# srbittner/torch_nf

Measured on AMD Instinct MI355X. Metric: M samples/sec NormFlow.log_prob, D=64 RealNVPx8, N=2^20, higher is better.
Workload: dtype f32

## Files before the change

torch_nf_amd/csrc/f16_tile2.h:

```cpp
#pragma once
#ifndef TNF2_ABL
#define TNF2_ABL 0
#endif
#if TNF2_ABL == 4
#define TNF_SPLIT_RNE_NO_REMAINDER 1
#endif
#include "f16_tile.h"
#include "support_math.h"

#ifndef TNF2_SCHED
#define TNF2_SCHED 0
#endif

namespace tnf {


typedef __bf16 bf2 __attribute__((ext_vector_type(2)));
typedef __bf16 bf8 __attribute__((ext_vector_type(8)));
typedef short s4 __attribute__((ext_vector_type(4)));
__device__ __forceinline__ unsigned pk_bf16(float a, float b) {
    return __builtin_bit_cast(unsigned, __builtin_convertvector(f2{a, b}, bf2));
}
__device__ __forceinline__ f4 mfma16b(u2 a, u2 b, f4 c) {
    return __builtin_amdgcn_mfma_f32_16x16x16bf16_1k(__builtin_bit_cast(s4, a), __builtin_bit_cast(s4, b), c, 0, 0, 0);
}
__device__ __forceinline__ f4 mfma32b(u4 a, u4 b, f4 c) {
    return __builtin_amdgcn_mfma_f32_16x16x32_bf16(__builtin_bit_cast(bf8, a), __builtin_bit_cast(bf8, b), c, 0, 0, 0);
}

__device__ __forceinline__ f4 contract16(u4 wv, h4 rh, h4 rl, f4 c) {
    const h4 wh = __builtin_bit_cast(h4, u2{wv[0], wv[1]}), wl = __builtin_bit_cast(h4, u2{wv[2], wv[3]});
    return mfma16h(wl, rh, mfma16h(wh, rl, mfma16h(wh, rh, c)));
}

__device__ __forceinline__ float sig2s(float a, float S) {
#if TNF2_ABL == 1
    return __builtin_fmaf(a, S, S);
#else
    return __builtin_amdgcn_rcpf(__builtin_fmaf(__builtin_amdgcn_exp2f(a), S, S));
#endif
}
__device__ __forceinline__ f4 sig2s_4(f4 v, float S) {
    return f4{sig2s(v[0], S), sig2s(v[1], S), sig2s(v[2], S), sig2s(v[3], S)};
}

template <int H, int L>
struct Img2 {
    static constexpr int HT = H / 16;
    static constexpr int N0 = (H == 32) ? 4 : 0;
    static constexpr int NK = ((H == 16) ? 2 : 0) + 2 * (L - 1) + 2 * HT;
    static constexpr int NBG = 2 + 2 * (L - 1) + 2 * HT;
    static constexpr int OFF_D = N0 * 256;
    static constexpr int OFF_B = OFF_D + NK * 256;
    static constexpr int OFF_S = OFF_B + NBG * 16;
    static constexpr int OFF_A = OFF_S + 8;
    static constexpr int FLOATS = OFF_A + 2 * H;
    __device__ static constexpr int k_l0(int net) { return net; }
    __device__ static constexpr int k_h(int l, int net) { return ((H == 16) ? 2 : 0) + 2 * l + net; }
    __device__ static constexpr int k_o(int net, int mo) { return ((H == 16) ? 2 : 0) + 2 * (L - 1) + net * HT + mo; }
    __device__ static constexpr int b_b0(int net) { return net; }
    __device__ static constexpr int b_bh(int l, int net) { return 2 + 2 * l + net; }
    __device__ static constexpr int b_b2(int net, int mo) { return 2 + 2 * (L - 1) + net * HT + mo; }
};
static_assert(Img2<32, 3>::FLOATS % 4 == 0 && Img2<16, 1>::FLOATS % 4 == 0, "images must stay 16-byte aligned");

template <int H>
__device__ __forceinline__ int layer_kappa(const float* __restrict__ p, int U, int lane, const float* foldc, int c,
                                           int din = H) {
    constexpr int D = 2 * H;
    constexpr int HT = H / 16;
    const int r = lane & 15, q = lane >> 4;
    const int coff = (c & 1) ? H : 0;
    const float* wt = p;
    const float* ws = p + din * U;
    float mx = 0.f;
#pragma unroll
    for (int m = 0; m < HT; ++m)
#pragma unroll
        for (int j = 0; j < 4; ++j) {
            const int f = 16 * m + 4 * q + j;
            const bool ok = r < U && f < din;
            const float a = foldc[coff + f];
            mx = fmaxf(mx, fabsf(kTwoLog2e * ld_sel(wt, f * U + r, ok) * a));
            mx = fmaxf(mx, fabsf(kTwoLog2e * ld_sel(ws, f * U + r, ok) * a));
        }
    (void)D;
    return pow2_norm(wave_max(mx), -30, 30);
}

template <int PREC>
__device__ __forceinline__ void store_k16(u4* gd, const float (&v)[4]) {
    if constexpr (PREC == 1) {
        *gd = u4{pk_bf16(v[0], v[1]), pk_bf16(v[2], v[3]), 0u, 0u};
    } else {
        const HiLo a = split2r(v[0], v[1]), b = split2r(v[2], v[3]);
        *gd = u4{a.hi, b.hi, a.lo, b.lo};
    }
}

template <int H, int L, int PREC = 0, bool FWD = false>
__device__ __forceinline__ void build_image2(float* img, const float* __restrict__ p, int U, int lane, const float* foldc,
                                             const float* foldprev, int c, float sc_in, float sc_prev, float sig_next,
                                             int din = H, int dout = H) {
    typedef Img2<H, L> I;
    constexpr int D = 2 * H;
    constexpr int HT = I::HT;
    LayerW<H, L> w;
    load_layer_w<H, L>(w, p, U, lane, din, dout);
    const int q = lane >> 4;
    const int coff = (c & 1) ? H : 0, toff = (c & 1) ? 0 : H;

#pragma unroll
    for (int net = 0; net < 2; ++net) {
        float pb = 0.f;
#pragma unroll
        for (int m = 0; m < HT; ++m)
#pragma unroll
            for (int j = 0; j < 4; ++j) {
                const int f = 16 * m + 4 * q + j;
                pb = __builtin_fmaf(w.w0[net][m * 4 + j], foldc[D + coff + f], pb);
                w.w0[net][m * 4 + j] *= foldc[coff + f] * sc_in;
            }
        pb = reduce_q(pb);
#pragma unroll
        for (int j = 0; j < 4; ++j) w.b0[net][j] += __shfl(pb, 4 * q + j);
    }
    float Sst[L][2];
#pragma unroll
    for (int l = 0; l < L - 1; ++l)
// ... 21 lines not shown
            if constexpr (FWD) w.b2[0][mo][j] *= sig_next;
            else w.b2[0][mo][j] = (w.b2[0][mo][j] - __builtin_fmaf(Ac, Bp, Bc)) * sig_next;
        }
#pragma unroll
    for (int net = 0; net < 2; ++net) {
        float mx = 0.f;
#pragma unroll
        for (int mo = 0; mo < HT; ++mo)
#pragma unroll
            for (int j = 0; j < 4; ++j) {
                if (net == 0) w.w2[0][mo][j] *= sig_next;
                mx = fmaxf(mx, fabsf(w.w2[net][mo][j]));
            }
        const float S = pow2i(pow2_norm(wave_max(mx), -15, 40));
        Sst[L - 1][net] = S;
#pragma unroll
        for (int mo = 0; mo < HT; ++mo)
#pragma unroll
            for (int j = 0; j < 4; ++j) w.w2[net][mo][j] *= S;
    }

    u4* g0 = reinterpret_cast<u4*>(img) + lane;
    u4* gd = reinterpret_cast<u4*>(img + I::OFF_D) + lane;
#pragma unroll
    for (int net = 0; net < 2; ++net) {
        if constexpr (H == 32) {
            u4 hi, lo;
#pragma unroll
            for (int pp = 0; pp < 4; ++pp) {
                if constexpr (PREC == 1) {
                    hi[pp] = pk_bf16(w.w0[net][2 * pp], w.w0[net][2 * pp + 1]);
                    lo[pp] = 0u;
                } else {
                    const HiLo s = split2r(w.w0[net][2 * pp], w.w0[net][2 * pp + 1]);
                    hi[pp] = s.hi;
                    lo[pp] = s.lo;
                }
            }
            g0[(2 * net) * 64] = hi;
            g0[(2 * net + 1) * 64] = lo;
        } else {
            const float v[4] = {w.w0[net][0], w.w0[net][1], w.w0[net][2], w.w0[net][3]};
            store_k16<PREC>(gd + I::k_l0(net) * 64, v);
        }
#pragma unroll
        for (int l = 0; l < L - 1; ++l) {
// ... 4 lines not shown
        for (int mo = 0; mo < HT; ++mo) {
            const float v[4] = {w.w2[net][mo][0], w.w2[net][mo][1], w.w2[net][mo][2], w.w2[net][mo][3]};
            store_k16<PREC>(gd + I::k_o(net, mo) * 64, v);
        }
    }
    if ((lane & 15) == 0) {
        float* bl = img + I::OFF_B + q * 4;
#pragma unroll
        for (int net = 0; net < 2; ++net) {
            *reinterpret_cast<f4*>(bl + I::b_b0(net) * 16) = w.b0[net];
#pragma unroll
            for (int l = 0; l < L - 1; ++l) *reinterpret_cast<f4*>(bl + I::b_bh(l, net) * 16) = w.bh[l][net];
#pragma unroll
            for (int mo = 0; mo < HT; ++mo) *reinterpret_cast<f4*>(bl + I::b_b2(net, mo) * 16) = w.b2[net][mo];
        }
#pragma unroll
        for (int mo = 0; mo < HT; ++mo) {
            *reinterpret_cast<f4*>(img + I::OFF_A + 16 * mo + 4 * q) = ays[mo];
            *reinterpret_cast<f4*>(img + I::OFF_A + H + 16 * mo + 4 * q) = bys[mo];
        }
    }
    if (lane == 0) {
#pragma unroll
        for (int l = 0; l < 4; ++l) {
            img[I::OFF_S + 2 * l] = l < L ? Sst[l < L ? l : 0][0] : 1.f;
            img[I::OFF_S + 2 * l + 1] = l < L ? Sst[l < L ? l : 0][1] : 1.f;
        }
    }
}

template <int H, int L, int NT>
__device__ __forceinline__ void coupling_tile2_bf16(const float* img, int lane, const f4 (&x)[NT][H / 16], f4 (&y)[NT][H / 16],
                                                    float (&ssum2)[NT]) {
    typedef Img2<H, L> I;
    constexpr int HT = I::HT;
    const u4* g0 = reinterpret_cast<const u4*>(img) + lane;
    const u4* gd = reinterpret_cast<const u4*>(img + I::OFF_D) + lane;
    const float* bl = img + I::OFF_B + (lane >> 4) * 4;
    auto bias = [&](int g) -> f4 { return *reinterpret_cast<const f4*>(bl + g * 16); };
    auto w16 = [&](int g) -> u2 { const u4 v = gd[g * 64]; return u2{v[0], v[1]}; };
    const f4 Sa = *reinterpret_cast<const f4*>(img + I::OFF_S);
    f4 Sb = {1.f, 1.f, 1.f, 1.f};
    if constexpr (L == 3) Sb = *reinterpret_cast<const f4*>(img + I::OFF_S + 4);
    auto Sc = [&](int stage, int net) -> float { return (2 * stage + net) < 4 ? Sa[2 * stage + net] : Sb[2 * stage + net - 4]; };
    auto b4 = [&](f4 v) -> u2 { return u2{pk_bf16(v[0], v[1]), pk_bf16(v[2], v[3])}; };

    f4 acc[NT][2];
// ... 24 lines not shown
        for (int t = 0; t < NT; ++t)
#pragma unroll
            for (int net = 0; net < 2; ++net) {
                acc[t][net] = mfma16b(w16(I::k_h(l, net)), rb[t][net], bias(I::b_bh(l, net)));
                rb[t][net] = b4(sig2s_4(acc[t][net], Sc(l + 1, net)));
            }
    }
#pragma unroll
    for (int mo = 0; mo < HT; ++mo) {
        const f4 ay = *reinterpret_cast<const f4*>(img + I::OFF_A + 16 * mo + 4 * (lane >> 4));
#pragma unroll
        for (int t = 0; t < NT; ++t) {
            const f4 tt = mfma16b(w16(I::k_o(0, mo)), rb[t][0], bias(I::b_b2(0, mo)));
            const f4 sv = mfma16b(w16(I::k_o(1, mo)), rb[t][1], bias(I::b_b2(1, mo)));
#pragma unroll
            for (int j = 0; j < 4; ++j) {
                ssum2[t] += sv[j];
                y[t][mo][j] = __builtin_fmaf(y[t][mo][j], ay[j], -tt[j]) * __builtin_amdgcn_exp2f(-sv[j]);
            }
        }
    }
}

template <int H, int L, int NT, bool SLOW, int PREC = 0, bool FWD = false>
__device__ __forceinline__ void coupling_tile2(const float* img, int lane, const f4 (&x)[NT][H / 16], f4 (&y)[NT][H / 16],
                                               float (&ssum2)[NT]) {
    static_assert(!(FWD && PREC == 1), "the bf16 experiment covers the inverse direction");
    if constexpr (PREC == 1) {
        coupling_tile2_bf16<H, L, NT>(img, lane, x, y, ssum2);
        return;
    }
    typedef Img2<H, L> I;
    constexpr int HT = I::HT;
#if TNF2_SCHED == 3 || TNF2_SCHED == 4
    __builtin_amdgcn_sched_barrier(0);
#elif TNF2_SCHED == 1
    __builtin_amdgcn_iglp_opt(0);
#elif TNF2_SCHED == 2
    __builtin_amdgcn_iglp_opt(1);
#endif
    const u4* g0 = reinterpret_cast<const u4*>(img) + lane;
    const u4* gd = reinterpret_cast<const u4*>(img + I::OFF_D) + lane;
    const float* bl = img + I::OFF_B + (lane >> 4) * 4;
    auto bias = [&](int g) -> f4 { return *reinterpret_cast<const f4*>(bl + g * 16); };
    const f4 Sa = *reinterpret_cast<const f4*>(img + I::OFF_S);
    f4 Sb = {1.f, 1.f, 1.f, 1.f};
    if constexpr (L == 3) Sb = *reinterpret_cast<const f4*>(img + I::OFF_S + 4);
    auto Sc = [&](int stage, int net) -> float { return (2 * stage + net) < 4 ? Sa[2 * stage + net] : Sb[2 * stage + net - 4]; };

    f4 acc[NT][2];
    if constexpr (!SLOW) {
        if constexpr (H == 32) {
            h8 xh[NT], xl[NT];
#pragma unroll
            for (int t = 0; t < NT; ++t) {
                const HiLo a = split2r(x[t][0][0], x[t][0][1]), b = split2r(x[t][0][2], x[t][0][3]);
                const HiLo c = split2r(x[t][1][0], x[t][1][1]), d = split2r(x[t][1][2], x[t][1][3]);
                xh[t] = __builtin_bit_cast(h8, u4{a.hi, b.hi, c.hi, d.hi});
                xl[t] = __builtin_bit_cast(h8, u4{a.lo, b.lo, c.lo, d.lo});
            }
#pragma unroll
            for (int net = 0; net < 2; ++net) {
                const h8 wh = __builtin_bit_cast(h8, g0[(2 * net) * 64]);
                const h8 wl = __builtin_bit_cast(h8, g0[(2 * net + 1) * 64]);
                const f4 b0 = bias(I::b_b0(net));
#pragma unroll
                for (int t = 0; t < NT; ++t) acc[t][net] = mfma32h(wh, xh[t], b0);
#pragma unroll
                for (int t = 0; t < NT; ++t) acc[t][net] = mfma32h(wh, xl[t], acc[t][net]);
#pragma unroll
                for (int t = 0; t < NT; ++t) acc[t][net] = mfma32h(wl, xh[t], acc[t][net]);
            }
        } else {
            h4 xh[NT], xl[NT];
#pragma unroll
            for (int t = 0; t < NT; ++t) split4r(x[t][0], xh[t], xl[t]);
#pragma unroll
            for (int net = 0; net < 2; ++net) {
                const u4 wv = gd[I::k_l0(net) * 64];
                const f4 b0 = bias(I::b_b0(net));
#pragma unroll
                for (int t = 0; t < NT; ++t) acc[t][net] = contract16(wv, xh[t], xl[t], b0);
            }
        }
    } else {
#pragma unroll
        for (int net = 0; net < 2; ++net) {
            float wv[H / 4];
            if constexpr (H == 32) {
                const h8 wh = __builtin_bit_cast(h8, g0[(2 * net) * 64]);
                const h8 wl = __builtin_bit_cast(h8, g0[(2 * net + 1) * 64]);
#pragma unroll
                for (int i = 0; i < 8; ++i) wv[i] = (float)wh[i] + (float)wl[i];
            } else {
                const h8 wd = __builtin_bit_cast(h8, gd[I::k_l0(net) * 64]);
#pragma unroll
                for (int i = 0; i < 4; ++i) wv[i] = (float)wd[i] + (float)wd[4 + i];
            }
            const f4 b0 = bias(I::b_b0(net));
// ... 4 lines not shown
#pragma unroll
                for (int t = 0; t < NT; ++t) acc[t][net] = mfma4(wv[i], x[t][i >> 2][i & 3], acc[t][net]);
        }
    }
    h4 rh[NT][2], rl[NT][2];
#pragma unroll
    for (int t = 0; t < NT; ++t)
#pragma unroll
        for (int net = 0; net < 2; ++net) split4r(sig2s_4(acc[t][net], Sc(0, net)), rh[t][net], rl[t][net]);
#pragma unroll
    for (int l = 0; l < L - 1; ++l) {
#pragma unroll
        for (int net = 0; net < 2; ++net) {
            const u4 wv = gd[I::k_h(l, net) * 64];
            const f4 bh = bias(I::b_bh(l, net));
#pragma unroll
            for (int t = 0; t < NT; ++t) acc[t][net] = contract16(wv, rh[t][net], rl[t][net], bh);
        }
#pragma unroll
        for (int t = 0; t < NT; ++t)
#pragma unroll
            for (int net = 0; net < 2; ++net) split4r(sig2s_4(acc[t][net], Sc(l + 1, net)), rh[t][net], rl[t][net]);
    }
#pragma unroll
    for (int mo = 0; mo < HT; ++mo) {
        f4 tt[NT], sv[NT];
        {
            const u4 wv = gd[I::k_o(0, mo) * 64];
            const f4 b2 = bias(I::b_b2(0, mo));
#pragma unroll
            for (int t = 0; t < NT; ++t) tt[t] = contract16(wv, rh[t][0], rl[t][0], b2);
        }
        {
            const u4 wv = gd[I::k_o(1, mo) * 64];
            const f4 b2 = bias(I::b_b2(1, mo));
#pragma unroll
            for (int t = 0; t < NT; ++t) sv[t] = contract16(wv, rh[t][1], rl[t][1], b2);
        }
        const f4 ay = *reinterpret_cast<const f4*>(img + I::OFF_A + 16 * mo + 4 * (lane >> 4));
        f4 by = {0.f, 0.f, 0.f, 0.f};
        if constexpr (FWD) by = *reinterpret_cast<const f4*>(img + I::OFF_A + H + 16 * mo + 4 * (lane >> 4));
#pragma unroll
        for (int t = 0; t < NT; ++t)
#pragma unroll
            for (int j = 0; j < 4; ++j) {
                const float s2 = sv[t][j];
#if TNF2_ABL == 3
                if (j == 0 && mo == 0) ssum2[t] += s2;
#else
                ssum2[t] += s2;
#endif
                if constexpr (FWD)
                    y[t][mo][j] = __builtin_fmaf(__builtin_fmaf(y[t][mo][j], ay[j], by[j]), __builtin_amdgcn_exp2f(s2), tt[t][j]);
                else
                    y[t][mo][j] = __builtin_fmaf(y[t][mo][j], ay[j], -tt[t][j]) * __builtin_amdgcn_exp2f(-s2);
            }
    }
#if TNF2_SCHED == 3 || TNF2_SCHED == 4
    constexpr int NMFMA = NT * 3 * (2 + 2 * (L - 1) + 2 * HT);
#pragma unroll
    for (int i = 0; i < NMFMA; ++i) {
        __builtin_amdgcn_sched_group_barrier(0x008, 1, 0);
#if TNF2_SCHED == 3
        __builtin_amdgcn_sched_group_barrier(0x002, 5, 0);
#else
        __builtin_amdgcn_sched_group_barrier(0x400, 2, 0);
        __builtin_amdgcn_sched_group_barrier(0x002, 3, 0);
#endif
    }
#endif
}

}
```

torch_nf_amd/csrc/flow_fused2.hip:

```cpp
#include <type_traits>

#include "f16_tile2.h"
#include "launch.h"

#ifndef TNF2_NT
#define TNF2_NT 2
#endif
#ifndef TNF2_NW
#define TNF2_NW 8
#endif
#ifndef TNF2_NW16
#define TNF2_NW16 12
#endif
#ifndef TNF2_RANGE_NT
#define TNF2_RANGE_NT 2
#endif
#ifndef TNF2_RANGE_NW
#define TNF2_RANGE_NW 8
#endif
#ifndef TNF2_RANGE_WGPC
#define TNF2_RANGE_WGPC 1
#endif
#ifndef TNF2_RANGE_ABL
#define TNF2_RANGE_ABL 0
// ... 12 lines not shown
#endif
#ifndef TNF2_RANGE_ALT
#define TNF2_RANGE_ALT 1
#endif
#ifndef TNF2_RANGE_NTMEM
#define TNF2_RANGE_NTMEM 2
#endif
#ifndef TNF2_FUSED_STAGE
#define TNF2_FUSED_STAGE 1
#endif
#ifndef TNF2_STAMP
#define TNF2_STAMP 0
#endif
#ifndef TNF2_UNROLL
#define TNF2_UNROLL 1
#endif
#ifndef TNF2_PAD_UNROLL32
#define TNF2_PAD_UNROLL32 0
#endif

namespace tnf {


template <int H, int L>
__host__ __device__ constexpr int flow2_lds_floats(int nl) {
    return nl * Img2<H, L>::FLOATS + (nl + 1) * 4 * H + 4 * H + ((nl + 3) / 4) * 4 + 4 + 16 + 7 * 2 * H;
}

template <int H, int L, int NT, int SS, bool SLOW, bool FWD = false>
__device__ __forceinline__ void run_layers2(const float* img, int S, int lane, f4 (&lo)[NT][H / 16], f4 (&hi)[NT][H / 16],
                                            float (&ssum)[NT]) {
    typedef Img2<H, L> I;
    if constexpr (FWD) {
        if constexpr (SS > 0 && !SLOW) {
#pragma unroll
            for (int st = 0; st < SS; ++st) {
                coupling_tile2<H, L, NT, false, 0, true>(img + (2 * st) * I::FLOATS, lane, lo, hi, ssum);
                coupling_tile2<H, L, NT, false, 0, true>(img + (2 * st + 1) * I::FLOATS, lane, hi, lo, ssum);
            }
        } else {
            for (int st = 0; st < S; ++st) {
                coupling_tile2<H, L, NT, SLOW, 0, true>(img + (2 * st) * I::FLOATS, lane, lo, hi, ssum);
                coupling_tile2<H, L, NT, SLOW, 0, true>(img + (2 * st + 1) * I::FLOATS, lane, hi, lo, ssum);
            }
        }
    } else if constexpr (SS > 0 && !SLOW) {
#pragma unroll
        for (int i = 0; i < SS; ++i) {
            const int st = SS - 1 - i;
            coupling_tile2<H, L, NT, false>(img + (2 * st + 1) * I::FLOATS, lane, hi, lo, ssum);
            coupling_tile2<H, L, NT, false>(img + (2 * st) * I::FLOATS, lane, lo, hi, ssum);
        }
    } else {
        for (int st = S - 1; st >= 0; --st) {
            coupling_tile2<H, L, NT, SLOW>(img + (2 * st + 1) * I::FLOATS, lane, hi, lo, ssum);
            coupling_tile2<H, L, NT, SLOW>(img + (2 * st) * I::FLOATS, lane, lo, hi, ssum);
        }
    }
}

__device__ __forceinline__ int pad_feature(int pf, int H, int h, int Dr) {
    if (pf < H) return pf < h ? pf : -1;
    return pf - H < Dr - h ? h + pf - H : -1;
}

template <int H, int L, int NT, int NWAVES, int SS = 0, bool FWD = false, bool PAD = false>
__global__ void __launch_bounds__(NWAVES * 64)
flow_fused2_kernel(Flow2Args a) {
    constexpr int D = 2 * H;
    constexpr int HT = H / 16;
    typedef Img2<H, L> I;
    const int Dr = PAD ? a.Dr : D;
    const int hr = Dr / 2;
    extern __shared__ __attribute__((aligned(16))) float lds[];
    const int nl = 2 * a.S;
    float* img = lds;
    float* fold = lds + nl * I::FLOATS;
    float* fin = fold + (nl + 1) * 2 * D;
    int* kap = reinterpret_cast<int*>(fin + 2 * D);
    int* qhead = kap + ((nl + 3) / 4) * 4;
    float* red = reinterpret_cast<float*>(qhead + 4);
    float* ivc = red + 16;
    float* stage = ivc + 7 * D;

    const int lane = threadIdx.x & 63;
    const int wave = threadIdx.x >> 6;
    const int s = lane & 15, q = lane >> 4;
    const int64_t m = grid_m();
    if (m >= (a.Mz > a.Mp ? a.Mz : a.Mp)) return;
    const int64_t mz = a.Mz == 1 ? 0 : m, mp = a.Mp == 1 ? 0 : m;
    const float* prow = a.params + mp * a.pstride;

    {
        float acc = 0.f;
// ... 28 lines not shown
        if constexpr (FWD)
            for (int i = threadIdx.x; i < 2 * D; i += NWAVES * 64) fold[i] = i < D ? 1.f : 0.f;
        acc = wave_sum(acc);
        if (lane == 0) red[wave] = acc;
        if (threadIdx.x == 0) *qhead = NWAVES;
        if (a.iv)
            for (int i = threadIdx.x; i < 7 * D; i += NWAVES * 64) ivc[i] = a.iv[i];
    }
    __syncthreads();
    auto d_cond = [&](int c) -> int { return PAD ? ((c & 1) ? Dr - hr : hr) : H; };
    auto d_tran = [&](int c) -> int { return PAD ? ((c & 1) ? hr : Dr - hr) : H; };
    for (int c = wave; c < nl; c += NWAVES) {
        const int kc = layer_kappa<H>(prow + (c >> 1) * a.stage_stride + (c & 1) * a.low_off, a.U, lane, fold + c * 2 * D, c,
                                      d_cond(c));
        if (lane == 0) kap[c] = kc;
    }
    __syncthreads();
    for (int c = wave; c < nl; c += NWAVES) {
        const float sc_in = pow2i(kap[c]);
        const float* pl = prow + (c >> 1) * a.stage_stride + (c & 1) * a.low_off;
        if constexpr (FWD) {
            const float sc_prev = c > 0 ? pow2i(kap[c - 1]) : 1.f;
            const float sig_next = c < nl - 1 ? pow2i(-kap[c + 1]) : 1.f;
            build_image2<H, L, 0, true>(img + c * I::FLOATS, pl, a.U, lane, fold + c * 2 * D,
                                        c > 0 ? fold + (c - 1) * 2 * D : nullptr, c, sc_in, sc_prev, sig_next, d_cond(c),
                                        d_tran(c));
        } else {
            const bool first = (c == nl - 1), last = (c == 0);
            const float sc_prev = first ? 1.f : pow2i(kap[c + 1]);
            const float sig_next = last ? 1.f : pow2i(-kap[c - 1]);
            build_image2<H, L>(img + c * I::FLOATS, pl, a.U, lane, fold + c * 2 * D,
                               first ? nullptr : fold + (c + 1) * 2 * D, c, sc_in, sc_prev, sig_next, d_cond(c), d_tran(c));
        }
    }
    if constexpr (FWD) {
        const float* fl = fold + nl * 2 * D;
        const float* fp = fold + (nl - 1) * 2 * D;
        const float sc = pow2i(kap[nl - 1]);
        for (int f = threadIdx.x; f < D; f += NWAVES * 64) {
            const bool up = f >= H;
            fin[f] = up ? fl[f] * fp[f] * sc : fl[f];
            fin[D + f] = up ? __builtin_fmaf(fl[f], fp[D + f], fl[D + f]) : fl[D + f];
        }
    } else {
        for (int f = threadIdx.x; f < H; f += NWAVES * 64) {
            fin[f] = fold[f] * pow2i(kap[0]);
            fin[D + f] = fold[D + f];
        }
    }
    const bool has_iv = !PAD && a.iv != nullptr;
    __syncthreads();

#if TNF2_PRIO
    if (__builtin_amdgcn_readfirstlane(threadIdx.x) >= 64 * (NWAVES / 2)) __builtin_amdgcn_s_setprio(1);
#endif
    const float presc = pow2i(-kap[FWD ? 0 : nl - 1]);
    const float* zb = a.z + mz * a.N * Dr;
    float* zo = a.z_out ? a.z_out + m * a.N * Dr : nullptr;
    float* sldo = a.sum_log_det ? a.sum_log_det + m * a.N : nullptr;
    float* lpo = a.log_prob ? a.log_prob + m * a.N : nullptr;
    float ldc = 0.f;
#pragma unroll
    for (int w = 0; w < NWAVES; ++w) ldc += red[w];

    const int64_t ngroups = (a.N + 16 * NT - 1) / (16 * NT);
    const int64_t per_block = (ngroups + gridDim.x - 1) / gridDim.x;
    const int64_t g_lo = (int64_t)blockIdx.x * per_block;
    const int64_t g_hi = (g_lo + per_block < ngroups) ? g_lo + per_block : ngroups;
    int64_t grp = g_lo + wave;
    if (grp >= g_hi) return;

    auto load_group = [&](int64_t g, f4 (&dlo)[NT][HT], f4 (&dhi)[NT][HT]) {
#pragma unroll
        for (int t = 0; t < NT; ++t) {
            int64_t row = (g * NT + t) * 16 + s;
            if (row >= a.N) row = a.N - 1;
            const float* zr = zb + row * D + 4 * q;
#pragma unroll
            for (int mm = 0; mm < HT; ++mm) {
                dlo[t][mm] = *reinterpret_cast<const f4*>(zr + 16 * mm);
                dhi[t][mm] = *reinterpret_cast<const f4*>(zr + H + 16 * mm);
            }
        }
    };
    constexpr int KR = D / 4;
    const int SP = Dr | 1;
// ... 93 lines not shown
#pragma unroll
                for (int t = 0; t < NT; ++t)
#pragma unroll
                    for (int j = 0; j < 4; ++j) dhi[t][mm][j] = __builtin_fmaf(dhi[t][mm][j], ga[j], gb[j]);
            }
        }
        if (FWD && has_iv) support(std::false_type{}, dlo, dhi, ssup);
    };

    f4 nlo[NT][HT], nhi[NT][HT];
    float nraw[NT][KR];
    if constexpr (PAD) load_raw(grp, nraw);
    else load_group(grp, nlo, nhi);
#if TNF2_STAMP
    const unsigned long long st_c0 = __builtin_amdgcn_s_memtime(), st_r0 = __builtin_amdgcn_s_memrealtime();
#endif

    for (;;) {
        int nxt_off = 0;
        if (lane == 0) nxt_off = atomicAdd(qhead, 1);
        const int64_t nxt = g_lo + __builtin_amdgcn_readfirstlane(nxt_off);
        const bool has_next = nxt < g_hi;
        f4 lo[NT][HT], hi[NT][HT];
        float ssum[NT], ssup[NT];
        if constexpr (PAD) unstage(nraw, lo, hi);
#pragma unroll
        for (int t = 0; t < NT; ++t) {
            ssum[t] = 0.f;
            ssup[t] = 0.f;
            if constexpr (!PAD)
#pragma unroll
                for (int mm = 0; mm < HT; ++mm) {
                    lo[t][mm] = nlo[t][mm];
                    hi[t][mm] = nhi[t][mm];
                }
        }
        double bsq[NT];
        if constexpr (FWD) {
#pragma unroll
            for (int t = 0; t < NT; ++t) {
                bsq[t] = 0.0;
                if (a.log_q) {
#pragma unroll
                    for (int mm = 0; mm < HT; ++mm)
#pragma unroll
                        for (int j = 0; j < 4; ++j) {
                            const double vl = (double)lo[t][mm][j], vh = (double)hi[t][mm][j];
                            bsq[t] = __builtin_fma(vl, vl, bsq[t]);
                            bsq[t] = __builtin_fma(vh, vh, bsq[t]);
                        }
                }
            }
        }
        enter(lo, hi, ssup);
        if (has_next) {
            if constexpr (PAD) load_raw(nxt, nraw);
            else load_group(nxt, nlo, nhi);
        }
        run_layers2<H, L, NT, SS, false, FWD>(img, a.S, lane, lo, hi, ssum);
        float chk = ssum[0];
#pragma unroll
        for (int t = 1; t < NT; ++t) chk += ssum[t];
        if (__builtin_expect(__any(chk != chk), 0)) {
            if constexpr (PAD) load_frag(grp, lo, hi);
            else load_group(grp, lo, hi);
#pragma unroll
            for (int t = 0; t < NT; ++t) {
                ssum[t] = 0.f;
                ssup[t] = 0.f;
            }
            enter(lo, hi, ssup);
            run_layers2<H, L, NT, 0, true, FWD>(img, a.S, lane, lo, hi, ssum);
            if (a.slow_count && lane == 0) atomicAdd(a.slow_count, 1u);
        }
        leave(lo, hi, ssup);
#pragma unroll
        for (int t = 0; t < NT; ++t) {
            const int64_t row = (grp * NT + t) * 16 + s;
            const bool row_ok = row < a.N;
            const float ld_tot = __builtin_fmaf(reduce_q(ssum[t]), kLn2, ldc) + (has_iv ? reduce_q(ssup[t]) : 0.f);
            if (!FWD && lpo) {
                float sq = 0.f;
#pragma unroll
                for (int mm = 0; mm < HT; ++mm)
#pragma unroll
                    for (int j = 0; j < 4; ++j) {
                        sq = __builtin_fmaf(lo[t][mm][j], lo[t][mm][j], sq);
                        sq = __builtin_fmaf(hi[t][mm][j], hi[t][mm][j], sq);
                    }
                sq = reduce_q(sq);
                if (q == 0 && row_ok) lpo[row] = -0.5f * sq - (float)Dr * 0.91893853320467274178f - ld_tot;
            }
            if (sldo && q == 0 && row_ok) sldo[row] = ld_tot;
            if constexpr (FWD) {
                if (a.log_q) {
                    double b = bsq[t];
                    b = reduce_q(b);
                    if (q == 0 && row_ok)
                        a.log_q[m * a.N + row] = (-0.5 * b - (double)Dr * 0.91893853320467274178) - (double)ld_tot;
                }
            }
            if (PAD && zo) {
                const int64_t row0 = (grp * NT + t) * 16;
// ... 564 lines not shown
#endif
                }
            } else {
                constexpr int LPR = H / 4, RPI = 64 / LPR;
                const int hoff = st_hi ? H : 0;
#pragma unroll
                for (int k = 0; k < NT * 16 / RPI; ++k) {
                    const int r = k * RPI + lane / LPR, ch = (hoff >> 2) + lane % LPR;
                    const f4 v = *reinterpret_cast<const f4*>(stg + sw_off(r, ch));
#if TNF2_RANGE_NTMEM & 2
                    if (row0 + r < a.N) __builtin_nontemporal_store(v, reinterpret_cast<f4*>(zo + (row0 + r) * D + (ch << 2)));
#else
                    if (row0 + r < a.N) *reinterpret_cast<f4*>(zo + (row0 + r) * D + (ch << 2)) = v;
#endif
                }
            }
        }
        if (!has_next) break;
        grp = nxt;
        if (STAGED && dma) stg = stg == stg0 ? stg0 + SLOT : stg0;
    }
}

template <int H, int L>
static size_t flow2_lds_bytes(int S) {
    return (size_t)flow2_lds_floats<H, L>(2 * S) * sizeof(float);
}

static size_t flow2_lds_bytes_rt(int D, int S, int L) {
    return dispatch_hl(D, L, [&](auto h, auto l) { return flow2_lds_bytes<h(), l()>(S); });
}

bool flow_fused2_supported(int D, int S, int L, int U) {
    if (!mfma_supported(D, L, U) || S < 1) return false;
    return flow2_lds_bytes_rt(D, S, L) <= 160 * 1024;
}

template <int H, int L, int NT, int NW, int SS, bool FWD, bool PAD = false>
static int launch2_t(const Flow2Args& a, int64_t M, hipStream_t st) {
    size_t smem = flow2_lds_bytes<H, L>(a.S);
    Flow2Args b = a;
    const size_t stage_bytes = (size_t)NW * 16 * 2 * H * sizeof(float);
    b.stage_out = (!PAD && H == 32 && a.z_out != nullptr && smem + stage_bytes <= 160 * 1024 && TNF2_FUSED_STAGE) ? 1 : 0;
    if (b.stage_out || PAD) smem += stage_bytes;
    const int64_t bx = persistent_bx_ceil((a.N + 16 * NT - 1) / (16 * NT), NW, 256, M);
    return launch_lds("flow_fused2", flow_fused2_kernel<H, L, NT, NW, SS, FWD, PAD>, grid_xm(bx, M), dim3(NW * 64), smem, st, b);
}

template <int H, int L, bool PAD = false>
static int launch2_v(const Flow2Args& a, int64_t M, int forward, hipStream_t st) {
    constexpr int NW = H == 16 ? TNF2_NW16 : TNF2_NW;
#if TNF2_UNROLL
    if (a.S == 4 && (!(PAD && H == 32) || TNF2_PAD_UNROLL32))
        return dispatch_bool(forward, [&](auto fwd) { return launch2_t<H, L, TNF2_NT, NW, 4, fwd(), PAD>(a, M, st); });
#endif
    return dispatch_bool(forward, [&](auto fwd) { return launch2_t<H, L, TNF2_NT, NW, 0, fwd(), PAD>(a, M, st); });
}

int launch_flow_fused2(const float* z, float* z0, float* sum_log_det, float* log_prob, int64_t Mz, int64_t Mp, int64_t N,
                       int D, int S, int L, int U, const float* params, int64_t pstride, const float* bn_mean,
                       const float* bn_alpha, const float* interval_consts, unsigned* slow_count, hipStream_t st,
                       int forward, double* log_q) {
    if (!flow_fused2_supported(D, S, L, U))
        return fail(TNF_EUNSUPPORTED, "flow_fused2: no kernel for D=%d S=%d L=%d U=%d", D, S, L, U);
    if (N <= 0) return TNF_OK;
    const int64_t M = Mz > Mp ? Mz : Mp;
    const FlowLayout fl = flow_layout(D, S, L, U);
    Flow2Args a = flow2_args(z, z0, sum_log_det, log_prob, Mz, Mp, N, S, U, params, pstride, bn_mean, bn_alpha, fl,
                             interval_consts, slow_count);
// ... 165 lines not shown
```

torch_nf_amd/csrc/wave_prims.h:

```cpp
#pragma once
#include <hip/hip_runtime.h>

#ifndef TNF_ABLATE
#define TNF_ABLATE 0
#endif
#ifndef TNF_SPLIT_RTZ_NO_REMAINDER
#define TNF_SPLIT_RTZ_NO_REMAINDER 0
#endif
#ifndef TNF_SPLIT_RNE_NO_REMAINDER
#define TNF_SPLIT_RNE_NO_REMAINDER 0
#endif

namespace tnf {

typedef float f2 __attribute__((ext_vector_type(2)));
typedef float f4 __attribute__((ext_vector_type(4)));
typedef _Float16 h2 __attribute__((ext_vector_type(2)));
typedef _Float16 h4 __attribute__((ext_vector_type(4)));
typedef _Float16 h8 __attribute__((ext_vector_type(8)));
typedef unsigned int u2 __attribute__((ext_vector_type(2)));
typedef unsigned int u4 __attribute__((ext_vector_type(4)));
typedef __attribute__((address_space(3))) void lds_void;

constexpr float kLog2e = 1.44269504088896340736f;
// ... 13 lines not shown
struct HiLo {
    unsigned hi, lo;
};
__device__ __forceinline__ void split_remainder(float& v0, float& v1, unsigned hb) {
    asm("v_fma_mix_f32 %0, %1, -1.0, %0 op_sel:[0,0,0] op_sel_hi:[1,0,0]" : "+v"(v0) : "v"(hb));
    asm("v_fma_mix_f32 %0, %1, -1.0, %0 op_sel:[1,0,0] op_sel_hi:[1,0,0]" : "+v"(v1) : "v"(hb));
}

__device__ __forceinline__ HiLo split2v(float v0, float v1) {
    const unsigned hb = __builtin_bit_cast(unsigned, __builtin_amdgcn_cvt_pkrtz(v0, v1));
#if TNF_SPLIT_RTZ_NO_REMAINDER
    return HiLo{hb, hb};
#endif
    split_remainder(v0, v1, hb);
    return HiLo{hb, __builtin_bit_cast(unsigned, __builtin_amdgcn_cvt_pkrtz(v0, v1))};
}
__device__ __forceinline__ HiLo split2r(float v0, float v1) {
    const unsigned hb = __builtin_bit_cast(unsigned, __builtin_convertvector(f2{v0, v1}, h2));
#if TNF_SPLIT_RNE_NO_REMAINDER
    return HiLo{hb, hb};
#endif
    split_remainder(v0, v1, hb);
    return HiLo{hb, __builtin_bit_cast(unsigned, __builtin_convertvector(f2{v0, v1}, h2))};
}
#define split2(V0, V1, HI, LO)                \
    do {                                      \
        const HiLo hl_ = split2v((V0), (V1)); \
        (HI) = hl_.hi;                        \
        (LO) = hl_.lo;                        \
    } while (0)

__device__ __forceinline__ void split4(f4 v, h4& hi, h4& lo) {
    const HiLo a = split2v(v[0], v[1]), b = split2v(v[2], v[3]);
    hi = __builtin_bit_cast(h4, u2{a.hi, b.hi});
    lo = __builtin_bit_cast(h4, u2{a.lo, b.lo});
}
__device__ __forceinline__ void split4r(f4 v, h4& hi, h4& lo) {
    const HiLo a = split2r(v[0], v[1]), b = split2r(v[2], v[3]);
    hi = __builtin_bit_cast(h4, u2{a.hi, b.hi});
    lo = __builtin_bit_cast(h4, u2{a.lo, b.lo});
}
__device__ __forceinline__ void split8(f4 v0, f4 v1, h8& hi, h8& lo) {
    const HiLo a = split2v(v0[0], v0[1]), b = split2v(v0[2], v0[3]);
    const HiLo c = split2v(v1[0], v1[1]), d = split2v(v1[2], v1[3]);
    hi = __builtin_bit_cast(h8, u4{a.hi, b.hi, c.hi, d.hi});
    lo = __builtin_bit_cast(h8, u4{a.lo, b.lo, c.lo, d.lo});
// ... 75 lines not shown
```

Measured before the change: 4577.

## Carry f16 hi/lo splits across coupling layers and add optional MFMA log-det path

In the inverse pass, each coupling layer now writes the f16 hi/lo split of its output into a packed buffer. The next layer reuses that buffer instead of re-splitting its conditioning input, and the split is done with inline fma_mix instructions. A second path, off by default, folds the log-det sum of the s-net outputs into an extra MFMA row in the weight image, replacing the per-element add chain. The packed buffers raise register pressure, and the hand-written assembly split adds maintenance risk.

```diff
diff --git a/torch_nf_amd/csrc/f16_tile2.h b/torch_nf_amd/csrc/f16_tile2.h
--- a/torch_nf_amd/csrc/f16_tile2.h
+++ b/torch_nf_amd/csrc/f16_tile2.h
@@ -5,8 +5,17 @@
 #if TNF2_ABL == 4
 #define TNF_SPLIT_RNE_NO_REMAINDER 1
 #endif
+#include <type_traits>
+
 #include "f16_tile.h"
 #include "support_math.h"
+
+#ifndef TNF2_PSPLIT
+#define TNF2_PSPLIT 1
+#endif
+#ifndef TNF2_LDMFMA
+#define TNF2_LDMFMA 0
+#endif
 
 #ifndef TNF2_SCHED
 #define TNF2_SCHED 0
@@ -44,11 +53,11 @@
     return f4{sig2s(v[0], S), sig2s(v[1], S), sig2s(v[2], S), sig2s(v[3], S)};
 }
 
-template <int H, int L>
+template <int H, int L, bool LDR = false>
 struct Img2 {
     static constexpr int HT = H / 16;
     static constexpr int N0 = (H == 32) ? 4 : 0;
-    static constexpr int NK = ((H == 16) ? 2 : 0) + 2 * (L - 1) + 2 * HT;
+    static constexpr int NK = ((H == 16) ? 2 : 0) + 2 * (L - 1) + 2 * HT + (LDR ? 1 : 0);
     static constexpr int NBG = 2 + 2 * (L - 1) + 2 * HT;
     static constexpr int OFF_D = N0 * 256;
     static constexpr int OFF_B = OFF_D + NK * 256;
@@ -58,11 +67,13 @@
     __device__ static constexpr int k_l0(int net) { return net; }
     __device__ static constexpr int k_h(int l, int net) { return ((H == 16) ? 2 : 0) + 2 * l + net; }
     __device__ static constexpr int k_o(int net, int mo) { return ((H == 16) ? 2 : 0) + 2 * (L - 1) + net * HT + mo; }
+    __device__ static constexpr int k_ld() { return NK - 1; }
     __device__ static constexpr int b_b0(int net) { return net; }
     __device__ static constexpr int b_bh(int l, int net) { return 2 + 2 * l + net; }
     __device__ static constexpr int b_b2(int net, int mo) { return 2 + 2 * (L - 1) + net * HT + mo; }
 };
 static_assert(Img2<32, 3>::FLOATS % 4 == 0 && Img2<16, 1>::FLOATS % 4 == 0, "images must stay 16-byte aligned");
+static_assert(Img2<32, 2, true>::FLOATS == Img2<32, 2>::FLOATS + 256, "the log-det row is one K = 16 group");
 
 template <int H>
 __device__ __forceinline__ int layer_kappa(const float* __restrict__ p, int U, int lane, const float* foldc, int c,
@@ -98,13 +109,14 @@
     }
 }
 
-template <int H, int L, int PREC = 0, bool FWD = false>
+template <int H, int L, int PREC = 0, bool FWD = false, bool LDR = false>
 __device__ __forceinline__ void build_image2(float* img, const float* __restrict__ p, int U, int lane, const float* foldc,
                                              const float* foldprev, int c, float sc_in, float sc_prev, float sig_next,
                                              int din = H, int dout = H) {
-    typedef Img2<H, L> I;
+    typedef Img2<H, L, LDR> I;
     constexpr int D = 2 * H;
     constexpr int HT = I::HT;
+    static_assert(!LDR || L <= 3, "the s-bias sum takes the scale slot of a fourth stage");
     LayerW<H, L> w;
     load_layer_w<H, L>(w, p, U, lane, din, dout);
     const int q = lane >> 4;
@@ -172,6 +184,26 @@
 
     u4* g0 = reinterpret_cast<u4*>(img) + lane;
     u4* gd = reinterpret_cast<u4*>(img + I::OFF_D) + lane;
+    if constexpr (LDR) {
+        float rs[4], sb = 0.f;
+#pragma unroll
+        for (int j = 0; j < 4; ++j) {
+            float c = 0.f;
+#pragma unroll
+            for (int mo = 0; mo < HT; ++mo) {
+                c += w.w2[1][mo][j];
+                sb += w.b2[1][mo][j];
+            }
+            c = row16_sum(c);
+            rs[j] = (lane & 15) == 0 ? c : 0.f;
+        }
+        store_k16<PREC>(gd + I::k_ld() * 64, rs);
+        sb = reduce_q(sb);
+        if (lane == 0) {
+            img[I::OFF_S + 6] = sb;
+            img[I::OFF_S + 7] = 0.f;
+        }
+    }
 #pragma unroll
     for (int net = 0; net < 2; ++net) {
         if constexpr (H == 32) {
@@ -222,7 +254,7 @@
     }
     if (lane == 0) {
 #pragma unroll
-        for (int l = 0; l < 4; ++l) {
+        for (int l = 0; l < (LDR ? 3 : 4); ++l) {
             img[I::OFF_S + 2 * l] = l < L ? Sst[l < L ? l : 0][0] : 1.f;
             img[I::OFF_S + 2 * l + 1] = l < L ? Sst[l < L ? l : 0][1] : 1.f;
         }
@@ -293,15 +325,36 @@
     }
 }
 
-template <int H, int L, int NT, bool SLOW, int PREC = 0, bool FWD = false>
+template <int H, int NT>
+struct Pk2 {
+    unsigned v[NT][2][H / 8];
+};
+template <int H, int NT>
+__device__ __forceinline__ void split_half(const f4 (&x)[NT][H / 16], Pk2<H, NT>& o) {
+#pragma unroll
+    for (int t = 0; t < NT; ++t)
+#pragma unroll
+        for (int m = 0; m < H / 16; ++m)
+#pragma unroll
+            for (int p = 0; p < 2; ++p) {
+                const HiLo a = split2r(x[t][m][2 * p], x[t][m][2 * p + 1]);
+                o.v[t][0][2 * m + p] = a.hi;
+                o.v[t][1][2 * m + p] = a.lo;
+            }
+}
+
+template <int H, int L, int NT, bool SLOW, int PREC = 0, bool FWD = false, class LD = float>
 __device__ __forceinline__ void coupling_tile2(const float* img, int lane, const f4 (&x)[NT][H / 16], f4 (&y)[NT][H / 16],
-                                               float (&ssum2)[NT]) {
+                                               LD (&ssum2)[NT], const Pk2<H, NT>* xs = nullptr, Pk2<H, NT>* ys = nullptr) {
     static_assert(!(FWD && PREC == 1), "the bf16 experiment covers the inverse direction");
+    constexpr bool LDR = std::is_same<LD, f4>::value;
+    static_assert(LDR || std::is_same<LD, float>::value, "log-det sum: float or accumulator tile");
     if constexpr (PREC == 1) {
+        static_assert(PREC != 1 || !LDR, "the bf16 experiment keeps the add chain");
         coupling_tile2_bf16<H, L, NT>(img, lane, x, y, ssum2);
         return;
     }
-    typedef Img2<H, L> I;
+    typedef Img2<H, L, LDR> I;
     constexpr int HT = I::HT;
 #if TNF2_SCHED == 3 || TNF2_SCHED == 4
     __builtin_amdgcn_sched_barrier(0);
@@ -325,6 +378,11 @@
             h8 xh[NT], xl[NT];
 #pragma unroll
             for (int t = 0; t < NT; ++t) {
+                if (xs) {
+                    xh[t] = __builtin_bit_cast(h8, u4{xs->v[t][0][0], xs->v[t][0][1], xs->v[t][0][2], xs->v[t][0][3]});
+                    xl[t] = __builtin_bit_cast(h8, u4{xs->v[t][1][0], xs->v[t][1][1], xs->v[t][1][2], xs->v[t][1][3]});
+                    continue;
+                }
                 const HiLo a = split2r(x[t][0][0], x[t][0][1]), b = split2r(x[t][0][2], x[t][0][3]);
                 const HiLo c = split2r(x[t][1][0], x[t][1][1]), d = split2r(x[t][1][2], x[t][1][3]);
                 xh[t] = __builtin_bit_cast(h8, u4{a.hi, b.hi, c.hi, d.hi});
@@ -345,7 +403,14 @@
         } else {
             h4 xh[NT], xl[NT];
 #pragma unroll
-            for (int t = 0; t < NT; ++t) split4r(x[t][0], xh[t], xl[t]);
+            for (int t = 0; t < NT; ++t) {
+                if (xs) {
+                    xh[t] = __builtin_bit_cast(h4, u2{xs->v[t][0][0], xs->v[t][0][1]});
+                    xl[t] = __builtin_bit_cast(h4, u2{xs->v[t][1][0], xs->v[t][1][1]});
+                } else {
+                    split4r(x[t][0], xh[t], xl[t]);
+                }
+            }
 #pragma unroll
             for (int net = 0; net < 2; ++net) {
                 const u4 wv = gd[I::k_l0(net) * 64];
@@ -396,6 +461,20 @@
 #pragma unroll
             for (int net = 0; net < 2; ++net) split4r(sig2s_4(acc[t][net], Sc(l + 1, net)), rh[t][net], rl[t][net]);
     }
+    auto ld_add = [&](int t, float s2, bool first) {
+        if constexpr (!LDR) {
+#if TNF2_ABL == 3
+            if (first)
+#endif
+                ssum2[t] += s2;
+        }
+        (void)first;
+    };
+    if constexpr (LDR) {
+        const u4 wv = gd[I::k_ld() * 64];
+#pragma unroll
+        for (int t = 0; t < NT; ++t) ssum2[t] = contract16(wv, rh[t][1], rl[t][1], ssum2[t]);
+    }
 #pragma unroll
     for (int mo = 0; mo < HT; ++mo) {
         f4 tt[NT], sv[NT];
@@ -414,16 +493,34 @@
         const f4 ay = *reinterpret_cast<const f4*>(img + I::OFF_A + 16 * mo + 4 * (lane >> 4));
         f4 by = {0.f, 0.f, 0.f, 0.f};
         if constexpr (FWD) by = *reinterpret_cast<const f4*>(img + I::OFF_A + H + 16 * mo + 4 * (lane >> 4));
+        if constexpr (!FWD) {
+            if (ys) {
+#pragma unroll
+                for (int t = 0; t < NT; ++t)
+#pragma unroll
+                    for (int p = 0; p < 2; ++p) {
+                        const int j0 = 2 * p, j1 = 2 * p + 1;
+                        ld_add(t, sv[t][j0], mo == 0 && p == 0);
+                        ld_add(t, sv[t][j1], false);
+                        float u0 = __builtin_fmaf(y[t][mo][j0], ay[j0], -tt[t][j0]);
+                        float u1 = __builtin_fmaf(y[t][mo][j1], ay[j1], -tt[t][j1]);
+                        const float v0 = u0 * __builtin_amdgcn_exp2f(-sv[t][j0]);
+                        const float v1 = u1 * __builtin_amdgcn_exp2f(-sv[t][j1]);
+                        y[t][mo][j0] = v0;
+                        y[t][mo][j1] = v1;
+                        const HiLo a = split2r_into(v0, v1, u0, u1);
+                        ys->v[t][0][2 * mo + p] = a.hi;
+                        ys->v[t][1][2 * mo + p] = a.lo;
+                    }
+                continue;
+            }
+        }
 #pragma unroll
         for (int t = 0; t < NT; ++t)
 #pragma unroll
             for (int j = 0; j < 4; ++j) {
                 const float s2 = sv[t][j];
-#if TNF2_ABL == 3
-                if (j == 0 && mo == 0) ssum2[t] += s2;
-#else
-                ssum2[t] += s2;
-#endif
+                ld_add(t, s2, mo == 0 && j == 0);
                 if constexpr (FWD)
                     y[t][mo][j] = __builtin_fmaf(__builtin_fmaf(y[t][mo][j], ay[j], by[j]), __builtin_amdgcn_exp2f(s2), tt[t][j]);
                 else
diff --git a/torch_nf_amd/csrc/flow_fused2.hip b/torch_nf_amd/csrc/flow_fused2.hip
--- a/torch_nf_amd/csrc/flow_fused2.hip
+++ b/torch_nf_amd/csrc/flow_fused2.hip
@@ -58,39 +58,61 @@
 namespace tnf {
 
 
-template <int H, int L>
+template <int H, int L, bool LDR = false>
 __host__ __device__ constexpr int flow2_lds_floats(int nl) {
-    return nl * Img2<H, L>::FLOATS + (nl + 1) * 4 * H + 4 * H + ((nl + 3) / 4) * 4 + 4 + 16 + 7 * 2 * H;
-}
-
-template <int H, int L, int NT, int SS, bool SLOW, bool FWD = false>
+    return nl * Img2<H, L, LDR>::FLOATS + (nl + 1) * 4 * H + 4 * H + ((nl + 3) / 4) * 4 + 4 + 16 + 7 * 2 * H;
+}
+
+template <int H, int L, bool PAD>
+constexpr bool kLeanBody2 = !PAD && !(H == 16 && L == 3);
+
+template <int H, int L, int NT, int SS, bool SLOW, bool FWD = false, class LD = float, bool PS = false>
 __device__ __forceinline__ void run_layers2(const float* img, int S, int lane, f4 (&lo)[NT][H / 16], f4 (&hi)[NT][H / 16],
-                                            float (&ssum)[NT]) {
-    typedef Img2<H, L> I;
+                                            LD (&ssum)[NT]) {
+    typedef Img2<H, L, std::is_same<LD, f4>::value> I;
     if constexpr (FWD) {
         if constexpr (SS > 0 && !SLOW) {
 #pragma unroll
             for (int st = 0; st < SS; ++st) {
-                coupling_tile2<H, L, NT, false, 0, true>(img + (2 * st) * I::FLOATS, lane, lo, hi, ssum);
-                coupling_tile2<H, L, NT, false, 0, true>(img + (2 * st + 1) * I::FLOATS, lane, hi, lo, ssum);
+                coupling_tile2<H, L, NT, false, 0, true, LD>(img + (2 * st) * I::FLOATS, lane, lo, hi, ssum);
+                coupling_tile2<H, L, NT, false, 0, true, LD>(img + (2 * st + 1) * I::FLOATS, lane, hi, lo, ssum);
             }
         } else {
             for (int st = 0; st < S; ++st) {
-                coupling_tile2<H, L, NT, SLOW, 0, true>(img + (2 * st) * I::FLOATS, lane, lo, hi, ssum);
-                coupling_tile2<H, L, NT, SLOW, 0, true>(img + (2 * st + 1) * I::FLOATS, lane, hi, lo, ssum);
-            }
+                coupling_tile2<H, L, NT, SLOW, 0, true, LD>(img + (2 * st) * I::FLOATS, lane, lo, hi, ssum);
+                coupling_tile2<H, L, NT, SLOW, 0, true, LD>(img + (2 * st + 1) * I::FLOATS, lane, hi, lo, ssum);
+            }
+        }
+    } else if constexpr (PS && !SLOW) {
+        Pk2<H, NT> pa, pb;
+        split_half<H, NT>(hi, pa);
+        if constexpr (SS > 0) {
+#pragma unroll
+            for (int i = 0; i < SS; ++i) {
+                const int st = SS - 1 - i;
+                coupling_tile2<H, L, NT, false, 0, false, LD>(img + (2 * st + 1) * I::FLOATS, lane, hi, lo, ssum, &pa, &pb);
+                coupling_tile2<H, L, NT, false, 0, false, LD>(img + (2 * st) * I::FLOATS, lane, lo, hi, ssum, &pb,
+                                                              st > 0 ? &pa : nullptr);
+            }
+        } else {
+            for (int st = S - 1; st > 0; --st) {
+                coupling_tile2<H, L, NT, false, 0, false, LD>(img + (2 * st + 1) * I::FLOATS, lane, hi, lo, ssum, &pa, &pb);
+                coupling_tile2<H, L, NT, false, 0, false, LD>(img + (2 * st) * I::FLOATS, lane, lo, hi, ssum, &pb, &pa);
+            }
+            coupling_tile2<H, L, NT, false, 0, false, LD>(img + I::FLOATS, lane, hi, lo, ssum, &pa, &pb);
+            coupling_tile2<H, L, NT, false, 0, false, LD>(img, lane, lo, hi, ssum, &pb);
         }
     } else if constexpr (SS > 0 && !SLOW) {
 #pragma unroll
         for (int i = 0; i < SS; ++i) {
             const int st = SS - 1 - i;
-            coupling_tile2<H, L, NT, false>(img + (2 * st + 1) * I::FLOATS, lane, hi, lo, ssum);
-            coupling_tile2<H, L, NT, false>(img + (2 * st) * I::FLOATS, lane, lo, hi, ssum);
+            coupling_tile2<H, L, NT, false, 0, false, LD>(img + (2 * st + 1) * I::FLOATS, lane, hi, lo, ssum);
+            coupling_tile2<H, L, NT, false, 0, false, LD>(img + (2 * st) * I::FLOATS, lane, lo, hi, ssum);
         }
     } else {
         for (int st = S - 1; st >= 0; --st) {
-            coupling_tile2<H, L, NT, SLOW>(img + (2 * st + 1) * I::FLOATS, lane, hi, lo, ssum);
-            coupling_tile2<H, L, NT, SLOW>(img + (2 * st) * I::FLOATS, lane, lo, hi, ssum);
+            coupling_tile2<H, L, NT, SLOW, 0, false, LD>(img + (2 * st + 1) * I::FLOATS, lane, hi, lo, ssum);
+            coupling_tile2<H, L, NT, SLOW, 0, false, LD>(img + (2 * st) * I::FLOATS, lane, lo, hi, ssum);
         }
     }
 }
@@ -100,12 +122,13 @@
     return pf - H < Dr - h ? h + pf - H : -1;
 }
 
-template <int H, int L, int NT, int NWAVES, int SS = 0, bool FWD = false, bool PAD = false>
+template <int H, int L, int NT, int NWAVES, int SS = 0, bool FWD = false, bool PAD = false, bool LDR = false>
 __global__ void __launch_bounds__(NWAVES * 64)
 flow_fused2_kernel(Flow2Args a) {
     constexpr int D = 2 * H;
     constexpr int HT = H / 16;
-    typedef Img2<H, L> I;
+    typedef Img2<H, L, LDR> I;
+    typedef typename std::conditional<LDR, f4, float>::type LD;
     const int Dr = PAD ? a.Dr : D;
     const int hr = Dr / 2;
     extern __shared__ __attribute__((aligned(16))) float lds[];
@@ -180,15 +203,16 @@
         if constexpr (FWD) {
             const float sc_prev = c > 0 ? pow2i(kap[c - 1]) : 1.f;
             const float sig_next = c < nl - 1 ? pow2i(-kap[c + 1]) : 1.f;
-            build_image2<H, L, 0, true>(img + c * I::FLOATS, pl, a.U, lane, fold + c * 2 * D,
-                                        c > 0 ? fold + (c - 1) * 2 * D : nullptr, c, sc_in, sc_prev, sig_next, d_cond(c),
-                                        d_tran(c));
+            build_image2<H, L, 0, true, LDR>(img + c * I::FLOATS, pl, a.U, lane, fold + c * 2 * D,
+                                             c > 0 ? fold + (c - 1) * 2 * D : nullptr, c, sc_in, sc_prev, sig_next, d_cond(c),
+                                             d_tran(c));
         } else {
             const bool first = (c == nl - 1), last = (c == 0);
             const float sc_prev = first ? 1.f : pow2i(kap[c + 1]);
             const float sig_next = last ? 1.f : pow2i(-kap[c - 1]);
-            build_image2<H, L>(img + c * I::FLOATS, pl, a.U, lane, fold + c * 2 * D,
-                               first ? nullptr : fold + (c + 1) * 2 * D, c, sc_in, sc_prev, sig_next, d_cond(c), d_tran(c));
+            build_image2<H, L, 0, false, LDR>(img + c * I::FLOATS, pl, a.U, lane, fold + c * 2 * D,
+                                              first ? nullptr : fold + (c + 1) * 2 * D, c, sc_in, sc_prev, sig_next, d_cond(c),
+                                              d_tran(c));
         }
     }
     if constexpr (FWD) {
@@ -220,6 +244,21 @@
     float ldc = 0.f;
 #pragma unroll
     for (int w = 0; w < NWAVES; ++w) ldc += red[w];
+    float sb_all = 0.f;
+    if constexpr (LDR)
+        for (int c = 0; c < nl; ++c) sb_all += img[c * I::FLOATS + I::OFF_S + 6];
+    auto ld_zero = [&]() -> LD {
+        if constexpr (LDR) return f4{sb_all, 0.f, 0.f, 0.f};
+        else return 0.f;
+    };
+    auto ld_raw = [&](const LD& v) -> float {
+        if constexpr (LDR) return v[0];
+        else return v;
+    };
+    auto ld_sum = [&](const LD& v) -> float {
+        if constexpr (LDR) return v[0];
+        else return reduce_q(v);
+    };
 
     const int64_t ngroups = (a.N + 16 * NT - 1) / (16 * NT);
     const int64_t per_block = (ngroups + gridDim.x - 1) / gridDim.x;
@@ -359,11 +398,12 @@
         const int64_t nxt = g_lo + __builtin_amdgcn_readfirstlane(nxt_off);
         const bool has_next = nxt < g_hi;
         f4 lo[NT][HT], hi[NT][HT];
-        float ssum[NT], ssup[NT];
+        LD ssum[NT];
+        float ssup[NT];
         if constexpr (PAD) unstage(nraw, lo, hi);
 #pragma unroll
         for (int t = 0; t < NT; ++t) {
-            ssum[t] = 0.f;
+            ssum[t] = ld_zero();
             ssup[t] = 0.f;
             if constexpr (!PAD)
 #pragma unroll
@@ -394,20 +434,20 @@
             if constexpr (PAD) load_raw(nxt, nraw);
             else load_group(nxt, nlo, nhi);
         }
-        run_layers2<H, L, NT, SS, false, FWD>(img, a.S, lane, lo, hi, ssum);
-        float chk = ssum[0];
-#pragma unroll
-        for (int t = 1; t < NT; ++t) chk += ssum[t];
+        run_layers2<H, L, NT, SS, false, FWD, LD, TNF2_PSPLIT && kLeanBody2<H, L, PAD>>(img, a.S, lane, lo, hi, ssum);
+        float chk = ld_raw(ssum[0]);
+#pragma unroll
+        for (int t = 1; t < NT; ++t) chk += ld_raw(ssum[t]);
         if (__builtin_expect(__any(chk != chk), 0)) {
             if constexpr (PAD) load_frag(grp, lo, hi);
             else load_group(grp, lo, hi);
 #pragma unroll
             for (int t = 0; t < NT; ++t) {
-                ssum[t] = 0.f;
+                ssum[t] = ld_zero();
                 ssup[t] = 0.f;
             }
             enter(lo, hi, ssup);
-            run_layers2<H, L, NT, 0, true, FWD>(img, a.S, lane, lo, hi, ssum);
+            run_layers2<H, L, NT, 0, true, FWD, LD>(img, a.S, lane, lo, hi, ssum);
             if (a.slow_count && lane == 0) atomicAdd(a.slow_count, 1u);
         }
         leave(lo, hi, ssup);
@@ -415,7 +455,7 @@
         for (int t = 0; t < NT; ++t) {
             const int64_t row = (grp * NT + t) * 16 + s;
             const bool row_ok = row < a.N;
-            const float ld_tot = __builtin_fmaf(reduce_q(ssum[t]), kLn2, ldc) + (has_iv ? reduce_q(ssup[t]) : 0.f);
+            const float ld_tot = __builtin_fmaf(ld_sum(ssum[t]), kLn2, ldc) + (has_iv ? reduce_q(ssup[t]) : 0.f);
             if (!FWD && lpo) {
                 float sq = 0.f;
 #pragma unroll
@@ -1026,9 +1066,9 @@
     }
 }
 
-template <int H, int L>
+template <int H, int L, bool LDR = false>
 static size_t flow2_lds_bytes(int S) {
-    return (size_t)flow2_lds_floats<H, L>(2 * S) * sizeof(float);
+    return (size_t)flow2_lds_floats<H, L, LDR>(2 * S) * sizeof(float);
 }
 
 static size_t flow2_lds_bytes_rt(int D, int S, int L) {
@@ -1040,15 +1080,21 @@
     return flow2_lds_bytes_rt(D, S, L) <= 160 * 1024;
 }
 
-template <int H, int L, int NT, int NW, int SS, bool FWD, bool PAD = false>
+template <int H, int L, int NT, int NW, int SS, bool FWD, bool PAD = false, bool LDR = false>
 static int launch2_t(const Flow2Args& a, int64_t M, hipStream_t st) {
     size_t smem = flow2_lds_bytes<H, L>(a.S);
     Flow2Args b = a;
     const size_t stage_bytes = (size_t)NW * 16 * 2 * H * sizeof(float);
     b.stage_out = (!PAD && H == 32 && a.z_out != nullptr && smem + stage_bytes <= 160 * 1024 && TNF2_FUSED_STAGE) ? 1 : 0;
     if (b.stage_out || PAD) smem += stage_bytes;
+    if constexpr (LDR || (TNF2_LDMFMA && kLeanBody2<H, L, PAD> && !FWD)) {
+        const size_t ldr_bytes = flow2_lds_bytes<H, L, true>(a.S) - flow2_lds_bytes<H, L, false>(a.S);
+        if constexpr (LDR) smem += ldr_bytes;
+        else if (smem + ldr_bytes <= 160 * 1024) return launch2_t<H, L, NT, NW, SS, FWD, PAD, true>(a, M, st);
+    }
     const int64_t bx = persistent_bx_ceil((a.N + 16 * NT - 1) / (16 * NT), NW, 256, M);
-    return launch_lds("flow_fused2", flow_fused2_kernel<H, L, NT, NW, SS, FWD, PAD>, grid_xm(bx, M), dim3(NW * 64), smem, st, b);
+    return launch_lds("flow_fused2", flow_fused2_kernel<H, L, NT, NW, SS, FWD, PAD, LDR>, grid_xm(bx, M), dim3(NW * 64), smem, st,
+                      b);
 }
 
 template <int H, int L, bool PAD = false>
diff --git a/torch_nf_amd/csrc/wave_prims.h b/torch_nf_amd/csrc/wave_prims.h
--- a/torch_nf_amd/csrc/wave_prims.h
+++ b/torch_nf_amd/csrc/wave_prims.h
@@ -59,6 +59,15 @@
 #endif
     split_remainder(v0, v1, hb);
     return HiLo{hb, __builtin_bit_cast(unsigned, __builtin_convertvector(f2{v0, v1}, h2))};
+}
+__device__ __forceinline__ HiLo split2r_into(float v0, float v1, float& d0, float& d1) {
+    const unsigned hb = __builtin_bit_cast(unsigned, __builtin_convertvector(f2{v0, v1}, h2));
+#if TNF_SPLIT_RNE_NO_REMAINDER
+    return HiLo{hb, hb};
+#endif
+    asm("v_fma_mix_f32 %0, %1, -1.0, %2 op_sel:[0,0,0] op_sel_hi:[1,0,0]" : "+v"(d0) : "v"(hb), "v"(v0));
+    asm("v_fma_mix_f32 %0, %1, -1.0, %2 op_sel:[1,0,0] op_sel_hi:[1,0,0]" : "+v"(d1) : "v"(hb), "v"(v1));
+    return HiLo{hb, __builtin_bit_cast(unsigned, __builtin_convertvector(f2{d0, d1}, h2))};
 }
 #define split2(V0, V1, HI, LO)                \
     do {                                      \
```

New measurement: 4699 (median of 6 runs). 1.03x the previous value.
